# zhejz/TrafficBotsV1.5

Hardware: NVIDIA B200
Metric: closed_loop_scenario_rollout_steps_per_sec (higher is better)
Workload: dtype tf32+fp16

## Files before the change

### trafficbotsv1.5_b200/csrc/ag_frontend.cu

```cuda
#include <cuda_fp16.h>

#include "common.cuh"

namespace {

constexpr int AW = 8;
constexpr int S1 = 32 + 8, S2 = 64 + 8, SP = 128 + 8;
constexpr int OFF_W1 = 0, OFF_W2 = OFF_W1 + 64 * S1, OFF_W3 = OFF_W2 + 64 * S2, OFF_P0 = OFF_W3 + 64 * S2,
              OFF_P1 = OFF_P0 + 64 * SP, OFF_P2 = OFF_P1 + 64 * SP, W_HALVES = OFF_P2 + 64 * SP;
constexpr int N_BIAS = 6 * 64;
constexpr size_t SMEM = (size_t)W_HALVES * 2 + (N_BIAS + 8) * 4;

__device__ __forceinline__ uint32_t pack_h2(float a, float b) { return tb_pack_h2_sat(a, b); }
__device__ __forceinline__ void mma16816(float (&d)[4], const uint32_t (&a)[4], uint32_t b0, uint32_t b1) {
  asm volatile(
      "mma.sync.aligned.m16n8k16.row.col.f32.f16.f16.f32 {%0,%1,%2,%3}, {%4,%5,%6,%7}, {%8,%9}, {%0,%1,%2,%3};"
      : "+f"(d[0]), "+f"(d[1]), "+f"(d[2]), "+f"(d[3])
      : "r"(a[0]), "r"(a[1]), "r"(a[2]), "r"(a[3]), "r"(b0), "r"(b1));
}

template <int KC>
__device__ __forceinline__ void dense64(const uint32_t (&a)[KC][4], const __half* __restrict__ Ws, int stride,
                                        const float* __restrict__ bias, int g, int t, float (&c)[8][4]) {
#pragma unroll
  for (int nt = 0; nt < 8; ++nt) {
    const float2 bb = *reinterpret_cast<const float2*>(bias + nt * 8 + 2 * t);
    c[nt][0] = bb.x; c[nt][1] = bb.y; c[nt][2] = bb.x; c[nt][3] = bb.y;
    const __half* wr = Ws + (nt * 8 + g) * stride + 2 * t;
#pragma unroll
    for (int kc = 0; kc < KC; ++kc)
      mma16816(c[nt], a[kc], *reinterpret_cast<const uint32_t*>(wr + kc * 16),
               *reinterpret_cast<const uint32_t*>(wr + kc * 16 + 8));
  }
}
template <bool RELU>
__device__ __forceinline__ void c_to_a(const float (&c)[8][4], uint32_t (*a)[4], uint32_t& hm) {
#pragma unroll
  for (int kc = 0; kc < 4; ++kc) {
    auto r = [](float v) { return RELU ? fmaxf(v, 0.f) : v; };
    a[kc][0] = pack_h2(r(c[2 * kc][0]), r(c[2 * kc][1]));
    a[kc][1] = pack_h2(r(c[2 * kc][2]), r(c[2 * kc][3]));
    a[kc][2] = pack_h2(r(c[2 * kc + 1][0]), r(c[2 * kc + 1][1]));
    a[kc][3] = pack_h2(r(c[2 * kc + 1][2]), r(c[2 * kc + 1][3]));
#pragma unroll
    for (int j = 0; j < 4; ++j) tb_track_h2(hm, a[kc][j]);
  }
}
__device__ __forceinline__ void relu_colmax(float (&c)[8][4], bool v_lo, bool v_hi, float (&m)[8][2]) {
#pragma unroll
  for (int nt = 0; nt < 8; ++nt) {
#pragma unroll
    for (int r = 0; r < 4; ++r) c[nt][r] = fmaxf(c[nt][r], 0.f);
    float a = fmaxf(v_lo ? c[nt][0] : -INFINITY, v_hi ? c[nt][2] : -INFINITY);
    float b = fmaxf(v_lo ? c[nt][1] : -INFINITY, v_hi ? c[nt][3] : -INFINITY);
#pragma unroll
    for (int o = 4; o < 32; o <<= 1) {
      a = fmaxf(a, __shfl_xor_sync(TB_FULL_MASK, a, o));
      b = fmaxf(b, __shfl_xor_sync(TB_FULL_MASK, b, o));
    }
    m[nt][0] = a; m[nt][1] = b;
  }
}
__device__ __forceinline__ float pe64(int c, float x, float y, float w, const float* __restrict__ f) {
  float a;
  bool is_sin;
  if (c < 16) { a = x * f[c & 7]; is_sin = c >= 8; }
  else if (c < 32) { a = y * f[c & 7]; is_sin = c >= 24; }
  else { a = w * (float)(((c - 32) & 15) + 1); is_sin = c >= 48; }
  return is_sin ? __sinf(a) : __cosf(a);
}

__global__ void __launch_bounds__(AW * 32, 2)
ag_frontend_kernel(const uint8_t* __restrict__ hist_valid, const float* __restrict__ hist_pose,
                   const float* __restrict__ hist_motion, const float* __restrict__ ag_attr,
                   const int* __restrict__ d_step, int step_stride, int A, const float* __restrict__ freq_xy,
                   int n_ag_tot, int W, const __half* __restrict__ wblob, const float* __restrict__ bias, float* __restrict__ tok_out,
                   int ldo, float* __restrict__ tok_pose, uint8_t* __restrict__ tok_invalid,
                   const float* __restrict__ ln_g, const float* __restrict__ ln_b, __half* __restrict__ ln_out,
                   int ld_ln, unsigned int* __restrict__ sat_flag) {
  extern __shared__ __align__(16) unsigned char smem[];
  __half* sW = reinterpret_cast<__half*>(smem);
  float* sB = reinterpret_cast<float*>(smem + (size_t)W_HALVES * 2);
  for (int i = threadIdx.x; i < W_HALVES / 8; i += blockDim.x)
    reinterpret_cast<uint4*>(sW)[i] = __ldg(reinterpret_cast<const uint4*>(wblob) + i);
  for (int i = threadIdx.x; i < N_BIAS; i += blockDim.x) sB[i] = __ldg(bias + i);
  if (threadIdx.x < 8) sB[N_BIAS + threadIdx.x] = __ldg(freq_xy + threadIdx.x);
  __syncthreads();

  const int warp = threadIdx.x >> 5, lane = threadIdx.x & 31;
  const int g = lane >> 2, t = lane & 3;
  const int s_all = *d_step;
  float* fr = sB + N_BIAS;
  uint32_t hm = 0u;

  for (int ba = blockIdx.x * AW + warp; ba < n_ag_tot; ba += gridDim.x * AW) {
    const size_t hb = (size_t)ba * W;
    const int s = step_stride ? d_step[(size_t)(ba / A) * step_stride] : s_all;
    const int n_step = min(s, W);
    int last_wp = -1;
    for (int wp = W - n_step; wp < W; ++wp)
      if (hist_valid[hb + ((s - W + wp) % W)]) last_wp = wp;
    float px = 0.f, py = 0.f, pw = 0.f;
    if (last_wp >= 0) {
      const int slot = (s - W + last_wp) % W;
      px = hist_pose[(hb + slot) * 3];
      py = hist_pose[(hb + slot) * 3 + 1];
      pw = hist_pose[(hb + slot) * 3 + 2];
    }
    if (lane == 0) {
      tok_pose[(size_t)ba * 3] = px; tok_pose[(size_t)ba * 3 + 1] = py; tok_pose[(size_t)ba * 3 + 2] = pw;
      tok_invalid[ba] = last_wp < 0;
    }
    float sn, cs;
    sincosf(pw, &sn, &cs);

    bool present[2], valid[2];
    float lx[2], ly[2], lw[2], mo[2][3];
#pragma unroll
    for (int h = 0; h < 2; ++h) {
      const int wp = g + 8 * h;
      present[h] = wp < W && wp >= W - n_step;
      const int slot = present[h] ? (s - W + wp) % W : 0;
      valid[h] = present[h] && hist_valid[hb + slot];
      lx[h] = ly[h] = lw[h] = 0.f;
      mo[h][0] = mo[h][1] = mo[h][2] = 0.f;
      if (present[h]) {
        const float* hp = hist_pose + (hb + slot) * 3;
        const float dx = hp[0] - px, dy = hp[1] - py;
        lx[h] = fmaf(dx, cs, dy * sn);
        ly[h] = fmaf(dy, cs, -dx * sn);
        lw[h] = hp[2] - pw;
        const float* hm = hist_motion + (hb + slot) * 3;
        mo[h][0] = hm[0]; mo[h][1] = hm[1]; mo[h][2] = hm[2];
      }
    }
    auto attr_el = [&](int h, int col) -> float {
      if (!present[h]) return 0.f;
      if (col < 6) return __ldg(ag_attr + (size_t)ba * 6 + col);
      if (col < 9) return col == 6 ? mo[h][0] : (col == 7 ? mo[h][1] : mo[h][2]);
      if (col < 9 + W) return (col - 9) == (g + 8 * h) ? 1.f : 0.f;
      return 0.f;
    };
    uint32_t a1[2][4];
#pragma unroll
    for (int kc = 0; kc < 2; ++kc) {
      const int c0 = 16 * kc + 2 * t;
      a1[kc][0] = pack_h2(attr_el(0, c0), attr_el(0, c0 + 1));
      a1[kc][1] = pack_h2(attr_el(1, c0), attr_el(1, c0 + 1));
      a1[kc][2] = pack_h2(attr_el(0, c0 + 8), attr_el(0, c0 + 9));
      a1[kc][3] = pack_h2(attr_el(1, c0 + 8), attr_el(1, c0 + 9));
    }
    float c[8][4];
    uint32_t x[8][4];
    dense64<2>(a1, sW + OFF_W1, S1, sB, g, t, c);
    c_to_a<true>(c, x, hm);
    {
      uint32_t a2[4][4];
#pragma unroll
      for (int kc = 0; kc < 4; ++kc)
#pragma unroll
        for (int r = 0; r < 4; ++r) a2[kc][r] = x[kc][r];
      dense64<4>(a2, sW + OFF_W2, S2, sB + 64, g, t, c);
      c_to_a<true>(c, a2, hm);
      dense64<4>(a2, sW + OFF_W3, S2, sB + 128, g, t, c);
      c_to_a<false>(c, x, hm);
    }
#pragma unroll
    for (int kc = 0; kc < 4; ++kc) {
      const int c0 = 16 * kc + 2 * t;
      x[4 + kc][0] = pack_h2(pe64(c0, lx[0], ly[0], lw[0], fr), pe64(c0 + 1, lx[0], ly[0], lw[0], fr));
      x[4 + kc][1] = pack_h2(pe64(c0, lx[1], ly[1], lw[1], fr), pe64(c0 + 1, lx[1], ly[1], lw[1], fr));
      x[4 + kc][2] = pack_h2(pe64(c0 + 8, lx[0], ly[0], lw[0], fr), pe64(c0 + 9, lx[0], ly[0], lw[0], fr));
      x[4 + kc][3] = pack_h2(pe64(c0 + 8, lx[1], ly[1], lw[1], fr), pe64(c0 + 9, lx[1], ly[1], lw[1], fr));
    }
    float m[8][2];
    dense64<8>(x, sW + OFF_P0, SP, sB + 192, g, t, c);
    relu_colmax(c, valid[0], valid[1], m);
#pragma unroll
    for (int layer = 1; layer < 3; ++layer) {
      c_to_a<false>(c, x, hm);
#pragma unroll
      for (int kc = 0; kc < 4; ++kc) {
        x[4 + kc][0] = x[4 + kc][1] = pack_h2(m[2 * kc][0], m[2 * kc][1]);
        x[4 + kc][2] = x[4 + kc][3] = pack_h2(m[2 * kc + 1][0], m[2 * kc + 1][1]);
      }
      dense64<8>(x, sW + (layer == 1 ? OFF_P1 : OFF_P2), SP, sB + 192 + 64 * layer, g, t, c);
      relu_colmax(c, valid[0], valid[1], m);
    }
    float2 o = make_float2(0.f, 0.f);
#pragma unroll
    for (int nt = 0; nt < 8; ++nt)
      if (nt == g) o = make_float2(m[nt][0], m[nt][1]);
    if (last_wp < 0) o = make_float2(0.f, 0.f);
    float* op = tok_out + (size_t)ba * ldo + 8 * g + 2 * t;
    *reinterpret_cast<float2*>(op) = o;
    *reinterpret_cast<float2*>(op + 64) = o;
    if (ln_out) {
      float sum = o.x + o.y;
#pragma unroll
      for (int of = 16; of; of >>= 1) sum += __shfl_xor_sync(TB_FULL_MASK, sum, of);
      const float mean = sum * (1.f / 64.f);
      const float dx = o.x - mean, dy = o.y - mean;
      float sq = fmaf(dx, dx, dy * dy);
#pragma unroll
      for (int of = 16; of; of >>= 1) sq += __shfl_xor_sync(TB_FULL_MASK, sq, of);
      const float rstd = 1.f / sqrtf(sq * (1.f / 64.f) + 1e-5f);
      const int c0 = 8 * g + 2 * t;
      __half* lp = ln_out + (size_t)ba * ld_ln + c0;
#pragma unroll
      for (int hlf = 0; hlf < 2; ++hlf) {
        const float2 gg = *reinterpret_cast<const float2*>(ln_g + c0 + 64 * hlf);
        const float2 bb = *reinterpret_cast<const float2*>(ln_b + c0 + 64 * hlf);
        *reinterpret_cast<__half2*>(lp + 64 * hlf) = __floats2half2_rn(dx * rstd * gg.x + bb.x, dy * rstd * gg.y + bb.y);
      }
    }
  }
  tb_flag_if_sat(hm, sat_flag);
}

}

extern "C" int tb_ag_frontend_blob_halves(void) { return W_HALVES; }

extern "C" int tb_ag_frontend_ex(const uint8_t* hist_valid, const float* hist_pose, const float* hist_motion,
                                 const float* ag_attr, const int* d_step, int step_stride, const float* freq_xy, int B,
                                 int A, int W, const void* wblob, const float* bias, float* tok_out, int ldo,
                                 float* tok_pose, uint8_t* tok_invalid, const float* ln_gamma, const float* ln_beta,
                                 void* ln_out, int ld_ln, void* stream) {
  if (!hist_valid || !hist_pose || !hist_motion || !ag_attr || !d_step || !freq_xy || !wblob || !bias || !tok_out ||
      !tok_pose || !tok_invalid)
    return TB_ERR_NULL;
  if (B <= 0 || A <= 0 || W <= 0 || ldo < 128 || step_stride < 0) return TB_ERR_BAD_SHAPE;
  if (W > 16 || 9 + W > 32) return TB_ERR_UNSUPPORTED;
  if ((ldo & 1) || !tb_aligned16(wblob) || (reinterpret_cast<uintptr_t>(tok_out) & 7)) return TB_ERR_MISALIGNED;
  if (ln_out) {
    if (!ln_gamma || !ln_beta) return TB_ERR_NULL;
    if (ld_ln < 128) return TB_ERR_BAD_SHAPE;
    if ((ld_ln & 1) || (reinterpret_cast<uintptr_t>(ln_out) & 3) || (reinterpret_cast<uintptr_t>(ln_gamma) & 7) ||
        (reinterpret_cast<uintptr_t>(ln_beta) & 7))
      return TB_ERR_MISALIGNED;
  }
  static bool attr_set = false;
  if (!attr_set) {
    if (cudaFuncSetAttribute(ag_frontend_kernel, cudaFuncAttributeMaxDynamicSharedMemorySize, (int)SMEM) != cudaSuccess)
      return TB_ERR_CUDA;
    attr_set = true;
  }
  static int num_sms = 0;
  if (num_sms == 0) {
    int dev = 0;
    cudaGetDevice(&dev);
    if (cudaDeviceGetAttribute(&num_sms, cudaDevAttrMultiProcessorCount, dev) != cudaSuccess || num_sms <= 0)
      num_sms = 148;
  }
  const int n = B * A;
  const int want = (n + AW - 1) / AW;
  const int grid = want < 2 * num_sms ? want : 2 * num_sms;
  ag_frontend_kernel<<<grid, AW * 32, SMEM, static_cast<cudaStream_t>(stream)>>>(
      hist_valid, hist_pose, hist_motion, ag_attr, d_step, step_stride, A, freq_xy, n, W,
      static_cast<const __half*>(wblob), bias, tok_out, ldo, tok_pose, tok_invalid, ln_gamma, ln_beta,
      static_cast<__half*>(ln_out), ld_ln, tb_fp16_flag_ptr);
  TB_CHECK_LAUNCH();
  return TB_OK;
}

extern "C" int tb_ag_frontend(const uint8_t* hist_valid, const float* hist_pose, const float* hist_motion,
                              const float* ag_attr, const int* d_step, const float* freq_xy, int B, int A, int W,
                              const void* wblob, const float* bias, float* tok_out, int ldo, float* tok_pose,
                              uint8_t* tok_invalid, const float* ln_gamma, const float* ln_beta, void* ln_out, int ld_ln,
                              void* stream) {
  return tb_ag_frontend_ex(hist_valid, hist_pose, hist_motion, ag_attr, d_step, 0, freq_xy, B, A, W, wblob, bias, tok_out,
                           ldo, tok_pose, tok_invalid, ln_gamma, ln_beta, ln_out, ld_ln, stream);
}
```

### trafficbotsv1.5_b200/model.py

```python
import math
from typing import Dict, Optional


import torch
from torch import Tensor

from . import ops

H = 4


def fuse_attention(P: Dict[str, Tensor], prefix: str, d: int, n_head: int = H, differentiable: bool = False
                   ) -> Dict[str, Tensor]:
    if differentiable:
        f64 = lambda k: P[f"{prefix}.{k}"].double()
    else:
        f64 = lambda k: P[f"{prefix}.{k}"].detach().double().cpu()
    w_in, b_in = f64("in_proj_weight"), f64("in_proj_bias")
    w_o, b_o = f64("out_proj_weight"), f64("out_proj_bias")
    w_r, b_r = f64("linear_rpe.weight"), f64("linear_rpe.bias")
    dh = d // n_head
    d_rpe = w_r.shape[1]
    s = math.log2(math.e) / math.sqrt(dh)
    w_q, b_q = w_in[:d] * s, b_in[:d] * s
    w_rk, w_rv, b_rv = w_r[:d], w_r[d:], b_r[d:]
    w_u, b_u, w_oz = [], [], []
    for h in range(n_head):
        sl = slice(h * dh, (h + 1) * dh)
        w_u.append(w_rk[sl].T @ w_q[sl])
        b_u.append(w_rk[sl].T @ b_q[sl])
        w_oz.append(w_o[:, sl] @ w_rv[sl])
    w_qu = torch.cat([w_q] + w_u, 0)
    b_qu = torch.cat([b_q] + b_u, 0)
    out = dict(
        w_in_self=torch.cat([w_qu, w_in[d:]], 0), b_in_self=torch.cat([b_qu, b_in[d:]], 0),
        w_in_q=w_qu, b_in_q=b_qu, w_kv=w_in[d:], b_kv=b_in[d:],
        w_out=torch.cat([w_o] + w_oz, 1), b_out=b_o + w_o @ b_rv,
    )
    return {k: v.float().contiguous() for k, v in out.items()}


def head_interleave_perm(d: int = 128, n_head: int = H) -> Tensor:
    assert d == 128 and n_head == 4
    s = torch.arange(d)
    head = 2 * (s >> 6) + ((s >> 3) & 1)
    return 32 * head + 8 * ((s >> 4) & 3) + (s & 7)


def _probe_fp32(fn):
    import functools

    @functools.wraps(fn)
    def wrapped(self, *a, **k):
        if getattr(self, "_probe_heads_fp32", False) and self.precision != 0:
            saved = (self.precision, self.kv_half)
            self.precision, self.kv_half = 0, False
            try:
                return fn(self, *a, **k)
            finally:
                self.precision, self.kv_half = saved
        return fn(self, *a, **k)
    return wrapped


class HotPathModel:

    _OPT = dict(attn_il=True, ln_fused=True, chain=True)

    @property
    def opt(self) -> dict:
        if "_opt" not in self.__dict__:
            self._opt = dict(self._OPT)
        return self._opt

    def __init__(self, P: Dict[str, Tensor], cfg: dict, sizes: dict, device="cuda", precision: int = 0):
        self.cfg, self.sz, self.dev, self.precision = cfg, sizes, torch.device(device), precision
        self.d = cfg["hidden_dim"]
        self.kv_half = precision == 1 and self.d == 128
        self.W = cfg["temp_window_size"]
        self.P = {k: v.detach().to(self.dev, torch.float32).contiguous() for k, v in P.items()}
        self.fa: Dict[str, Dict[str, Tensor]] = {}
        for k in P:
            if k.endswith(".in_proj_weight"):
                p = k[: -len(".in_proj_weight")]
                self.fa[p] = {n: t.to(self.dev) for n, t in fuse_attention(P, p, self.d).items()}
        self.freq_rpe = ops.pe_freq_xy(self.d, cfg["pose_rpe"]["theta_xy"], self.dev)
        self.freq_ag = ops.pe_freq_xy(self.d // 2, cfg["ag_encoder"]["pose_emb"]["theta_xy"], self.dev)
        self.act_w0 = torch.cat([self.P[f"action_head.mlp_mean.{t}.fc_layers.0.weight"] for t in range(3)], 0)
        self.act_b0 = torch.cat([self.P[f"action_head.mlp_mean.{t}.fc_layers.0.bias"] for t in range(3)], 0)
        self.act_w4 = torch.block_diag(*[self.P[f"action_head.mlp_mean.{t}.fc_layers.4.weight"] for t in range(3)]
                                       ).contiguous()
        self.act_b4 = torch.cat([self.P[f"action_head.mlp_mean.{t}.fc_layers.4.bias"] for t in range(3)], 0)

    @classmethod
    def from_state_dict(cls, sd: Dict[str, Tensor], d_model: int, theta_xy: float = 1e3, device="cuda",
                        precision: int = 0) -> "HotPathModel":
        self = cls.__new__(cls)
        self.cfg, self.sz, self.dev, self.precision = None, None, torch.device(device), precision
        self.d, self.W = d_model, None
        self.kv_half = precision == 1 and d_model == 128
        self.P = {k: v.detach().to(self.dev, torch.float32).contiguous() for k, v in sd.items()}
        self.fa = {}
        for k in sd:
            if k.endswith("in_proj_weight"):
                p = k[: -len(".in_proj_weight")] if k.endswith(".in_proj_weight") else ""
                P = sd if p else {f".{n}": t for n, t in sd.items()}
                self.fa[p] = {n: t.to(self.dev) for n, t in fuse_attention(P, p, d_model).items()}
        self.freq_rpe = ops.pe_freq_xy(d_model, theta_xy, self.dev)
        return self

    @property
    def gp(self) -> int:
        return 3 if (self.precision == 0 and getattr(self, "fp32_tc", True)) else self.precision

    def lin(self, x, wname, relu=False, **kw):
        return ops.linear(x, self.P[f"{wname}.weight"], self.P[f"{wname}.bias"], relu=relu, precision=self.gp,
                          **kw)

    def ln(self, x, name, half: bool = False):
        return ops.layernorm(x, self.P[f"{name}.weight"], self.P[f"{name}.bias"],
                             out_dtype=torch.float16 if half else torch.float32)

    @property
    def kv_il(self) -> bool:
        return self.kv_half and self.opt["attn_il"]

    def _proj(self, x: Tensor, key: str, w: Tensor, b: Tensor, il_blocks=(), **kw):
        if x.dtype == torch.float16:
            if il_blocks and self.kv_il:
                w, b = self._interleaved(key, w, b, il_blocks)
                key += ".il"
            return ops.linear(x, self._half(key, w), b, precision=2, **kw)
        return ops.linear(x, w, b, precision=self.gp, **kw)

    def _interleaved(self, key: str, w: Tensor, b: Tensor, blocks):
        if not hasattr(self, "_w_il"):
            self._w_il = {}
        if key not in self._w_il:
            rows = torch.arange(w.shape[0], device=w.device)
            perm = head_interleave_perm(self.d).to(w.device)
            for r0 in blocks:
                rows[r0:r0 + self.d] = r0 + perm
            self._w_il[key] = (w[rows].contiguous(), b[rows].contiguous())
        return self._w_il[key]

    def mlp(self, x, prefix, idxs, end_act, **last_kw):
        for n, i in enumerate(idxs):
            last = n == len(idxs) - 1
            x = self.lin(x, f"{prefix}.fc_layers.{i}", relu=(not last) or end_act, **(last_kw if last else {}))
        return x

    def pointnet(self, x: Tensor, row_invalid: Tensor, G: int, Lg: int, prefix: str) -> Tensor:
        half = self.d // 2
        h = self.lin(x, f"{prefix}.mlp_layers.0.fc_layers.0", relu=True)
        for i in (1, 2):
            m = ops.pointnet_pool(h, row_invalid, G, Lg, 1)
            w_l, w_r = self._pointnet_split(prefix, i)
            gb = ops.linear(m, w_r, self.P[f"{prefix}.mlp_layers.{i}.fc_layers.0.bias"], precision=self.gp)
            h = ops.linear(h, w_l, gb, relu=True, bias_group=Lg, precision=self.gp)
        return ops.pointnet_pool(h, row_invalid, G, Lg, 2)

    def _pointnet_split(self, prefix: str, i: int):
        key = f"{prefix}.{i}"
        if not hasattr(self, "_pn_split"):
            self._pn_split = {}
        if key not in self._pn_split:
            w = self.P[f"{prefix}.mlp_layers.{i}.fc_layers.0.weight"]
            half = w.shape[1] // 2
            self._pn_split[key] = (w[:, :half].contiguous(), w[:, half:].contiguous())
        return self._pn_split[key]

    def kv_table(self, feat: Tensor, layer_prefix: str, norm: str, attn: str = "attn", out: Optional[Tensor] = None
                 ) -> Tensor:
        f = self.fa[f"{layer_prefix}.{attn}"]
        x = self.ln(feat, f"{layer_prefix}.{norm}", half=self.kv_half)
        if self.kv_half:
            tbl = out if out is not None else torch.empty(x.shape[0], 2 * self.d, dtype=torch.float16, device=x.device)
            self._proj(x, f"{layer_prefix}.{attn}.w_kv", f["w_kv"], f["b_kv"], out_h=tbl, col_h=0,
                       il_blocks=(0, self.d))
            return tbl
        return ops.linear(x, f["w_kv"], f["b_kv"], precision=self.gp, out=out)

    def _in_self(self, f, x, K, key=""):
        nq = self.d + H * self.d
        if self.kv_half:
            row = torch.empty(x.shape[0], nq + 2 * self.d, dtype=torch.float16, device=x.device)
            self._proj(x, f"{key}.w_in_self", f["w_in_self"], f["b_in_self"], out_h=row, col_h=0,
                       il_blocks=(0, nq, nq + self.d))
            return row[:, :nq], row[:, nq:]
        proj = ops.linear(x, f["w_in_self"], f["b_in_self"], precision=self.gp)
        return proj, proj[:, nq:]

    def _in_q(self, f, x, key=""):
        if self.kv_half:
            qu = torch.empty(x.shape[0], self.d + H * self.d, dtype=torch.float16, device=x.device)
            self._proj(x, f"{key}.w_in_q", f["w_in_q"], f["b_in_q"], out_h=qu, col_h=0, il_blocks=(0,))
            return qu
        return ops.linear(x, f["w_in_q"], f["b_in_q"], precision=self.gp)

    def _attend(self, fa, proj, B, S, kv0, T0, div0, K0, knn, kv1=None, T1=0, div1=1, K1=0):
        d = self.d
        if torch.is_grad_enabled() and any(t is not None and t.requires_grad for t in (proj, kv0, kv1)):
            from . import autograd as AG
            return AG.knarpe_attn(proj[:, :d + H * d], kv0, T0, div0, K0, knn["idx"], knn["inv"], knn["rel"],
                                  self.freq_rpe, B, S, d, H, kv1=kv1, T1=T1, div1=div1, K1=K1,
                                  fast_trig=self.precision == 1)
        return ops.knarpe_attn(proj[:, :d], proj[:, d:d + H * d], kv0, T0, div0, K0, knn["idx"], knn["inv"],
                               knn.get("rel"), self.freq_rpe, B, S, d, H, kv1=kv1, T1=T1, div1=div1, K1=K1,
                               emb=knn.get("emb"), fast_trig=self.precision == 1, interleaved=self.kv_il,
                               out_dtype=torch.float16 if self.kv_half else torch.float32)

    def _half(self, key: str, w: Tensor) -> Tensor:
        if not hasattr(self, "_w_half"):
            self._w_half = {}
        if key not in self._w_half:
            self._w_half[key] = w.to(torch.float16).contiguous()
        return self._w_half[key]

    @property
    def chain_fused(self) -> bool:
        return self.opt["chain"]

    def _ffn_program(self, p: str, ldy: int, ln_next: Optional[str]):
        if not hasattr(self, "_chain"):
            self._chain = {}
        key = ("ffn", p, ldy, ln_next)
        if key not in self._chain:
            d = self.d
            w1 = self._half(f"{p}.linear1", self.P[f"{p}.linear1.weight"])
            w2 = self._half(f"{p}.linear2", self.P[f"{p}.linear2.weight"])
            nh = w1.shape[0] // d
            assert w1.shape == (nh * d, d) and w2.shape == (d, nh * d) and nh <= 4
            q = ops.ChainProgram(self.dev, n_buf=nh)
            q.load(0, d, 0, f16=True)
            hb = [(t + 1) % nh for t in range(nh)]
            for t in range(nh):
                q.gemm(w1, [0], self.P[f"{p}.linear1.bias"], n0=t * d, relu=True, out_buf=hb[t])
            ln = dict(ln_out=4, ld_ln=d, ln_gamma=self.P[f"{ln_next}.weight"], ln_beta=self.P[f"{ln_next}.bias"]) if ln_next else {}
            q.gemm(w2, hb, self.P[f"{p}.linear2.bias"], res=1, ldr=d, mask_post=2, out_g=3, ldg=ldy, **ln)
            self._chain[key] = q.finish()
        return self._chain[key]

    def _heads_program(self):
        if not hasattr(self, "_chain"):
            self._chain = {}
        if "heads" not in self._chain:
            d = self.d
            hw = lambda n: self._half(n, self.P[f"{n}.weight"])
            b = lambda n: self.P[f"{n}.bias"]
            q = ops.ChainProgram(self.dev, n_buf=4)
            q.load(1, d, 1)
            q.load(0, 2 * d, 0)
            n = "navi_encoder.mlp_pe.fc_layers.0"
            q.gemm(hw(n), [1], b(n), res=2, ldr=d, out_buf=2)
            for i, (src_b, dst_b) in zip((0, 3, 6), ((2, 1), (1, 2), (2, 1))):
                n = f"add_navi.mlp_in.fc_layers.{i}"
                q.gemm(hw(n), [src_b], b(n), relu=True, out_buf=dst_b, mask_post=3 if i == 6 else -1)
            n = "add_navi.mlp.fc_layers.0"
            q.gemm(hw(n), [0, 1], b(n), relu=True, out_buf=2)
            n = "add_navi.mlp.fc_layers.3"
            q.gemm(hw(n), [2], b(n), relu=True, out_buf=3)
            n = "add_navi.mlp.fc_layers.6"
            q.gemm(hw(n), [3], b(n), relu=True, mask_pre=3, res=0, ldr=2 * d, out_buf=0, out_g=4, ldg=2 * d)
            q.load(4, 2 * d, 1, src_col=d)
            n = "add_latent.mlp.fc_layers.0"
            q.gemm(hw(n), [0, 1], b(n), relu=True, out_buf=2)
            n = "add_latent.mlp.fc_layers.3"
            q.gemm(hw(n), [2], b(n), relu=True, out_buf=3)
            n = "add_latent.mlp.fc_layers.6"
            q.gemm(hw(n), [3], b(n), relu=True, mask_pre=5, res=4, ldr=2 * d, out_buf=0)
            w0 = self._half("action_head.w0", self.act_w0)
            for t in range(3):
                q.gemm(w0, [0], self.act_b0, n0=t * d, relu=True, out_buf=1 + t)
            for t in range(3):
                n = f"action_head.mlp_mean.{t}.fc_layers.2"
                q.gemm(hw(n), [1 + t], b(n), relu=True, out_buf=1 + t)
            q.gemm(self._half("action_head.w4", self.act_w4), [1, 2, 3], self.act_b4, out_g=6, ldg=6, n_valid=6)
            self._chain["heads"] = q.finish()
        return self._chain["heads"]

    @property
    def ln_fused(self) -> bool:
        return self.kv_half and self.d == 128 and self.opt["ln_fused"]

    def _out_proj(self, p: str, f: dict, o: Tensor, nv: Tensor, res: Tensor, ln_next: Optional[str] = None):
        if o.dtype == torch.float16:
            w = self._half(f"{p}.w_out", f["w_out"])
            if ln_next is not None and self.ln_fused:
                return ops.linear_ln(o, w, f["b_out"], self.P[f"{ln_next}.weight"], self.P[f"{ln_next}.bias"], mask_pre=nv,
                                     res=res, precision=2)
            y = ops.linear(o, w, f["b_out"], mask_pre=nv, res=res, precision=2)
        else:
            y = ops.linear(o, f["w_out"], f["b_out"], mask_pre=nv, res=res, precision=self.gp)
        return y if ln_next is None else (y, self.ln(y, ln_next, half=self.kv_half))

    def tf_layer(self, p: str, mode: str, src: Tensor, src_inv: Tensor, B: int, S: int, knn_self: dict,
                 cross: Optional[dict] = None, out: Optional[Tensor] = None, before_self=None, before_cross=None,
                 ln_in: Optional[Tensor] = None, ln_next: Optional[str] = None):
        d, pr = self.d, self.precision
        if mode == "dec_cross_attn":
            f = self.fa[f"{p}.attn_src"]
            x0 = ln_in if ln_in is not None else self.ln(src, f"{p}.norm_src", half=self.kv_half)
            proj, kv = self._in_self(f, x0, knn_self["idx"].shape[-1], f"{p}.attn_src")
            if before_self is not None:
                before_self()
            o, nv = self._attend(f, proj, B, S, kv, S, 1, knn_self["idx"].shape[-1], knn_self)
            src, x1 = self._out_proj(f"{p}.attn_src", f, o, nv, src, ln_next=f"{p}.norm1")
            f = self.fa[f"{p}.attn"]
            proj = self._in_q(f, x1, f"{p}.attn")
            if before_cross is not None:
                before_cross()
            o, nv = self._attend(f, proj, B, S, cross["kv0"], cross["T0"], cross["div0"], cross["K0"], cross,
                                 cross.get("kv1"), cross.get("T1", 0), cross.get("div1", 1), cross.get("K1", 0))
            src, x2 = self._out_proj(f"{p}.attn", f, o, nv, src, ln_next=f"{p}.norm2")
        else:
            f = self.fa[f"{p}.attn"]
            x0 = ln_in if ln_in is not None else self.ln(src, f"{p}.norm1", half=self.kv_half)
            proj, kv = self._in_self(f, x0, knn_self["idx"].shape[-1], f"{p}.attn")
            o, nv = self._attend(f, proj, B, S, kv, S, 1, knn_self["idx"].shape[-1], knn_self)
            src, x2 = self._out_proj(f"{p}.attn", f, o, nv, src, ln_next=f"{p}.norm2")
        if self.kv_half:
            h = torch.empty(x2.shape[0], self.P[f"{p}.linear1.weight"].shape[0], dtype=torch.float16, device=x2.device)
            self._proj(x2, f"{p}.linear1", self.P[f"{p}.linear1.weight"], self.P[f"{p}.linear1.bias"], relu=True, out_h=h,
                       col_h=0)
            w2 = self._half(f"{p}.linear2", self.P[f"{p}.linear2.weight"])
            if ln_next is not None and self.ln_fused:
                return ops.linear_ln(h, w2, self.P[f"{p}.linear2.bias"], self.P[f"{ln_next}.weight"],
                                     self.P[f"{ln_next}.bias"], res=src, mask_post=src_inv, out=out, precision=2)
            y = ops.linear(h, w2, self.P[f"{p}.linear2.bias"], res=src, mask_post=src_inv, out=out, precision=2)
        else:
            h = self.lin(x2, f"{p}.linear1", relu=True)
            y = self.lin(h, f"{p}.linear2", res=src, mask_post=src_inv, out=out)
        return y if ln_next is None else (y, self.ln(y, ln_next, half=self.kv_half))

    def tf_stack(self, prefix: str, n_layer: int, mode: str, tok: Tensor, layer_kw, ln_in: Optional[Tensor] = None
                 ) -> Tensor:
        first = "norm_src" if mode == "dec_cross_attn" else "norm1"
        for i in range(n_layer):
            args, kw = layer_kw(i)
            nxt = f"{prefix}.{i + 1}.{first}" if (i + 1 < n_layer and self.ln_fused) else None
            r = self.tf_layer(f"{prefix}.{i}", mode, tok, *args, ln_in=ln_in, ln_next=nxt, **kw)
            tok, ln_in = r if nxt is not None else (r, None)
        return tok

    def map_encoder(self, mp_valid: Tensor, mp_attr: Tensor, mp_pose: Tensor) -> Dict[str, Tensor]:
        d, sz = self.d, self.sz
        n_sc, n_mp, Ln = mp_valid.shape
        tok_pose = mp_pose[:, :, 0].contiguous()
        tok_inv = ~mp_valid[:, :, 0]
        c, s = torch.cos(tok_pose[..., 2]), torch.sin(tok_pose[..., 2])
        rot = torch.stack([torch.stack([c, -s], -1), torch.stack([s, c], -1)], -2)
        xy = torch.matmul(mp_pose[..., :2] - tok_pose[:, :, None, :2], rot)
        yaw = mp_pose[..., 2] - tok_pose[..., 2:3]
        pe7 = _encode_polyline(xy, torch.stack([yaw.cos(), yaw.sin()], -1))
        attr = torch.cat([mp_attr[:, :, None, :].expand(-1, -1, Ln, -1),
                          torch.eye(Ln, device=self.dev)[None, None].expand(n_sc, n_mp, -1, -1)], -1)
        M = n_sc * n_mp * Ln
        x = torch.empty(M, d, device=self.dev)
        x[:, d - 7:] = pe7.reshape(M, 7)
        self.mlp(attr.reshape(M, -1).contiguous(), "mp_encoder.input_encoder.mlp", (0, 2, 4), False, out=x[:, : d - 7])
        tok = self.pointnet(x, (~mp_valid).reshape(-1).contiguous(), n_sc * n_mp, Ln, "mp_encoder.pl_encoder")
        idx, inv, rel = ops.knn_select(tok_pose, tok_inv, tok_pose, tok_inv, sz["k_mp2mp"], sz["dl_mp"])
        knn = dict(idx=idx, inv=inv, rel=rel)
        flat_inv = tok_inv.reshape(-1).contiguous()
        tok = self.tf_stack("mp_encoder.tf_mp2mp.layers", self.cfg["mp_encoder"]["n_layer_tf"], "enc_self_attn", tok,
                            lambda i: ((flat_inv, n_sc, n_mp, knn), {}))
        return dict(mp_token_invalid=tok_inv.contiguous(), mp_token_feature=tok.view(n_sc, n_mp, d),
                    mp_token_pose=tok_pose, knn_mp2mp=knn, **self.sorted_map(tok_pose, tok_inv))

    @staticmethod
    def sorted_map(tok_pose: Tensor, tok_inv: Tensor) -> Dict[str, Tensor]:
        order = torch.argsort(tok_pose[..., 0], dim=1)
        return dict(mp_sorted_pose=torch.gather(tok_pose, 1, order[..., None].expand(-1, -1, 3)).contiguous(),
                    mp_sorted_invalid=torch.gather(tok_inv, 1, order).contiguous(),
                    mp_sorted_index=order.to(torch.int32).contiguous())

    def tl_pre_compute(self, tl_valid: Tensor, tl_attr: Tensor, tl_pose: Tensor, mp: Dict[str, Tensor]) -> dict:
        sz, d = self.sz, self.d
        n_sc, n_tl = tl_valid.shape
        n_mp = mp["mp_token_pose"].shape[1]
        inv = (~tl_valid).contiguous()
        tl_pose = tl_pose.contiguous()
        feat2d = mp["mp_token_feature"].reshape(n_sc * n_mp, d)
        attr = ops.gather_rows(mp["mp_token_feature"].contiguous(), tl_attr.to(torch.int32).reshape(-1).contiguous(),
                               n_tl)
        i1, m1, r1 = ops.knn_select(tl_pose, inv, tl_pose, inv, sz["k_tl2tl"], sz["dl_tl"])
        i2, m2, r2 = ops.knn_select(tl_pose, inv, mp["mp_token_pose"], mp["mp_token_invalid"], sz["k_tl2mp"],
                                    sz["dl_tl"])
        kv = [self.kv_table(feat2d, f"tl_encoder.tf_tl2tlmp.layers.{i}", "norm_tgt")
              for i in range(self.cfg["tl_encoder"]["n_layer_tf"])]
        W = self.W
        return dict(tl_token_invalid=inv, tl_token_pose=tl_pose, tl_token_attr=attr,
                    tl_attr_rows=attr.view(n_sc * n_tl, 1, d).expand(-1, W, -1).reshape(-1, d).contiguous(),
                    knn_self=dict(idx=i1, inv=m1, rel=r1),
                    cross=[dict(kv0=kv[i], T0=n_mp, div0=1, K0=sz["k_tl2mp"], idx=i2, inv=m2, rel=r2)
                           for i in range(len(kv))], n_sc=n_sc, n_tl=n_tl)

    def tl_forward(self, hist_tl: Tensor, d_step: Tensor, tl: dict, out_feat: Optional[Tensor] = None,
                   out_logits: Optional[Tensor] = None, with_logits: bool = True):
        from . import lib as L
        Bt, n_tl, W, d = tl["n_sc"], tl["n_tl"], self.W, self.d
        M = Bt * n_tl * W
        attr = torch.empty(M, 5 + W, device=self.dev)
        row_inv = torch.empty(M, dtype=torch.bool, device=self.dev)
        L.check(L.load().tb_tl_featurize_ex(L.ptr(hist_tl), L.ptr(ops._u8(tl["tl_token_invalid"])), L.ptr(d_step),
                                            1 if d_step.numel() > 1 else 0, Bt, n_tl, W, L.ptr(attr), 5 + W,
                                            L.ptr(ops._u8(row_inv)), L.stream()), "tb_tl_featurize_ex")
        ops._count()
        x = self.mlp(attr, "tl_encoder.input_encoder.mlp", (0, 2, 4), False, res=tl["tl_attr_rows"])
        tok = self.pointnet(x, row_inv, Bt * n_tl, W, "tl_encoder.temp_encoder")
        flat_inv = tl["tl_token_invalid"].reshape(-1)
        nl = self.cfg["tl_encoder"]["n_layer_tf"]
        tok = self.tf_stack("tl_encoder.tf_tl2tlmp.layers", nl, "dec_cross_attn", tok,
                            lambda i: ((flat_inv, Bt, n_tl, tl["knn_self"], tl["cross"][i]),
                                       dict(out=out_feat if i == nl - 1 else None)))
        if not with_logits:
            return tok, None
        tok_in = tok.detach() if getattr(self, "detach_tl_feature", False) else tok
        logits = self.mlp(tok_in, "tl_state_predictor.mlp", (0, 2, 4), False, out=out_logits)
        return tok, logits

    def ag_static(self, mp: Dict[str, Tensor]) -> list:
        n_sc, n_mp, d = mp["mp_token_feature"].shape
        feat2d = mp["mp_token_feature"].reshape(n_sc * n_mp, d)
        return [self.kv_table(feat2d, f"ag_encoder.tf_ag2agmptl.layers.{i}", "norm_tgt")
                for i in range(self.cfg["ag_encoder"]["n_layer_tf"])]

    def ag_forward(self, st: dict, mp: Dict[str, Tensor], kv_mp: list, tl: dict, tl_feat: Tensor, R: int,
                   out: Optional[Tensor] = None, aux: Optional[dict] = None, before_tl=None, knn_stream=None,
                   knn_stream2=None, kv_tl: Optional[list] = None, tl_pose_div: Optional[int] = None) -> Tensor:
        from . import lib as L
        sz, d, W = self.sz, self.d, self.W
        B, A = st["B"], st["A"]
        n_mp, n_tl = mp["mp_token_pose"].shape[1], tl["n_tl"]
        tl_div = B // (tl_feat.shape[0] // n_tl)
        M, MW = B * A, B * A * W
        tok_pose = torch.empty(B, A, 3, device=self.dev)
        tok_inv = torch.empty(B, A, dtype=torch.bool, device=self.dev)
        fused = self.kv_half and W <= 16 and d == 128
        hist = (L.ptr(st["hist_valid"]), L.ptr(st["hist_pose"]), L.ptr(st["hist_motion"]), L.ptr(st["ag_attr"]),
                L.ptr(st["d_step"]), L.ptr(self.freq_ag), B, A, W)
        per_row_step = st["d_step"].numel() > 1
        stride = 1 if per_row_step else 0
        if fused:
            L.check(L.load().tb_ag_featurize_ex(*hist[:5], stride, *hist[5:], L.ptr(tok_pose), L.ptr(ops._u8(tok_inv)),
                                                None, None, 0, None, 0, L.stream()), "tb_ag_featurize_ex")
        else:
            row_inv = torch.empty(MW, dtype=torch.bool, device=self.dev)
            attr = torch.empty(MW, 9 + W, device=self.dev)
            x = torch.empty(MW, d, device=self.dev)
            L.check(L.load().tb_ag_featurize_ex(*hist[:5], stride, *hist[5:], L.ptr(tok_pose),
                                                L.ptr(ops._u8(tok_inv)), L.ptr(ops._u8(row_inv)), L.ptr(attr), 9 + W,
                                                L.ptr(x[:, d // 2:]), d, L.stream()), "tb_ag_featurize_ex")
        ops._count()
        Kc, Ka = sz["k_ag2mp"] + sz["k_ag2tl"], sz["k_ag2ag"]
        i_aa = torch.empty(B, A, Ka, dtype=torch.int32, device=self.dev)
        m_aa = torch.empty(B, A, Ka, dtype=torch.bool, device=self.dev)
        r_aa = torch.empty(B, A, Ka, 3, device=self.dev)
        cidx = torch.empty(B, A, Kc, dtype=torch.int32, device=self.dev)
        cinv = torch.empty(B, A, Kc, dtype=torch.bool, device=self.dev)
        crel = torch.empty(B, A, Kc, 3, device=self.dev)

        def select_self():
            ops.knn_select(tok_pose, tok_inv, tok_pose, tok_inv, Ka, sz["dl_ag"], out=(i_aa, m_aa, r_aa))

        def select_cross():
            if "knn_state" in st and "mp_sorted_pose" in mp:
                ops.knn_select(tok_pose, tok_inv, mp["mp_sorted_pose"], mp["mp_sorted_invalid"], sz["k_ag2mp"],
                               sz["dl_ag"], tgt_div=R, out=(cidx, cinv, crel), koff=0,
                               index_map=mp["mp_sorted_index"], row_state=st["knn_state"], sorted_by_x=True)
            else:
                ops.knn_select(tok_pose, tok_inv, mp["mp_token_pose"], mp["mp_token_invalid"], sz["k_ag2mp"],
                               sz["dl_ag"], tgt_div=R, out=(cidx, cinv, crel), koff=0)
            ops.knn_select(tok_pose, tok_inv, tl["tl_token_pose"], tl["tl_token_invalid"], sz["k_ag2tl"], sz["dl_ag"],
                           tgt_div=tl_pose_div or tl_div, out=(cidx, cinv, crel), koff=sz["k_ag2mp"],
                           row_state=st.get("knn_state_tl"))

        main = torch.cuda.current_stream()
        join_self = join_cross = None
        if knn_stream is not None:
            s2 = knn_stream2 if knn_stream2 is not None else knn_stream
            s2.wait_stream(main)
            with torch.cuda.stream(s2):
                select_self()
            knn_stream.wait_stream(main)
            with torch.cuda.stream(knn_stream):
                select_cross()
            join_self = lambda: main.wait_stream(s2)
            join_cross = lambda: main.wait_stream(knn_stream)
        if fused:
            blob, bias = self._ag_frontend_weights()
            tok = torch.empty(M, d, device=self.dev)
            tp2, ti2 = torch.empty_like(tok_pose), torch.empty_like(tok_inv)
            ln0 = None
            if self.ln_fused:
                ln0 = torch.empty(M, d, dtype=torch.float16, device=self.dev)
                nm = "ag_encoder.tf_ag2agmptl.layers.0.norm_src"
                ln_args = (L.ptr(self.P[f"{nm}.weight"]), L.ptr(self.P[f"{nm}.bias"]), L.ptr(ln0), d)
            else:
                ln_args = (None, None, None, 0)
            L.check(L.load().tb_ag_frontend_ex(*hist[:5], stride, *hist[5:], L.ptr(blob), L.ptr(bias), L.ptr(tok), d,
                                               L.ptr(tp2), L.ptr(ops._u8(ti2)), *ln_args, L.stream()),
                    "tb_ag_frontend_ex")
            ops._count()
        else:
            ln0 = None
            self.mlp(attr, "ag_encoder.input_encoder.mlp", (0, 2, 4), False, out=x[:, : d // 2])
            tok = self.pointnet(x, row_inv, M, W, "ag_encoder.temp_encoder")
        if knn_stream is None:
            select_self()
            select_cross()
        knn_self = dict(idx=i_aa, inv=m_aa, rel=r_aa)
        flat_inv = tok_inv.reshape(-1)
        nl = self.cfg["ag_encoder"]["n_layer_tf"]
        if aux is not None:
            aux.update(tok_pose=tok_pose, tok_inv=tok_inv, tok0=tok, knn_self=knn_self, cidx=cidx, cinv=cinv, crel=crel)
        if before_tl is not None and kv_tl is None:
            before_tl()

        def join_first_cross():
            if join_cross is not None:
                join_cross()
            if before_tl is not None and kv_tl is not None:
                before_tl()

        def layer_kw(i):
            p = f"ag_encoder.tf_ag2agmptl.layers.{i}"
            kv1 = kv_tl[i] if kv_tl is not None else self.kv_table(tl_feat, p, "norm_tgt")
            cross = dict(kv0=kv_mp[i], T0=n_mp, div0=R, K0=sz["k_ag2mp"], kv1=kv1, T1=n_tl, div1=tl_div,
                         K1=sz["k_ag2tl"], idx=cidx, inv=cinv, rel=crel)
            return (flat_inv, B, A, knn_self, cross), dict(out=out if i == nl - 1 else None,
                                                           before_self=join_self if i == 0 else None,
                                                           before_cross=join_first_cross if i == 0 else None)

        tok = self.tf_stack("ag_encoder.tf_ag2agmptl.layers", nl, "dec_cross_attn", tok, layer_kw, ln_in=ln0)
        return tok

    def ag_tl_tables(self, tl_feat: Tensor, out: Optional[list] = None) -> list:
        return [self.kv_table(tl_feat, f"ag_encoder.tf_ag2agmptl.layers.{i}", "norm_tgt",
                              out=out[i] if out is not None else None)
                for i in range(self.cfg["ag_encoder"]["n_layer_tf"])]

    def navi_predictor(self, ag_valid: Tensor, ag_attr: Tensor, ag_motion: Tensor, ag_pose: Tensor,
                       mp: Dict[str, Tensor], ag_type: Tensor, mp_type: Tensor, scene_chunk: int = 4) -> Tensor:
        d, W = self.d, self.W
        n_sc, A, n_step = ag_valid.shape
        if n_step > W:
            ag_valid, ag_motion, ag_pose, n_step = ag_valid[:, :, -W:], ag_motion[:, :, -W:], ag_pose[:, :, -W:], W
        tok_valid = ag_valid.any(-1)
        last = n_step - 1 - torch.max(ag_valid.flip(2).to(torch.uint8), dim=2)[1]
        tok_pose = torch.gather(ag_pose, 2, last[:, :, None, None].expand(-1, -1, 1, 3)).squeeze(2)
        tok_pose = tok_pose.masked_fill(~tok_valid[..., None], 0.0).contiguous()
        M, MW = n_sc * A, n_sc * A * n_step
        attr = torch.cat([ag_attr[:, :, None, :].expand(-1, -1, n_step, -1), ag_motion,
                          torch.eye(W, device=self.dev)[None, None, -n_step:].expand(n_sc, A, -1, -1)], -1)
        x = torch.empty(MW, d, device=self.dev)
        self.mlp(attr.reshape(MW, -1).contiguous(), "navi_predictor.input_encoder.mlp", (0, 2, 4), False,
                 out=x[:, : d // 2])
        ops.pose_emb(ag_pose.reshape(MW, 3), self.freq_ag, d // 2, frame=tok_pose, frame_div=n_step, out=x[:, d // 2:])
        tok = self.pointnet(x, (~ag_valid).reshape(-1).contiguous(), M, n_step, "navi_predictor.temp_encoder")
        pr = "navi_predictor.mlp.fc_layers"
        w0 = self.P[f"{pr}.0.weight"]
        a_part = ops.linear(tok, w0[:, :d].contiguous(), self.P[f"{pr}.0.bias"], precision=self.gp)
        w_mr = w0[:, d:].contiguous()
        n_mp = mp["mp_token_pose"].shape[1]
        logits = torch.empty(n_sc, A, n_mp, device=self.dev)
        for s0 in range(0, n_sc, scene_chunk):
            ns = min(scene_chunk, n_sc - s0)
            Pn = ns * A * n_mp
            X = torch.empty(Pn, 2 * d, device=self.dev)
            X[:, :d].view(ns, A, n_mp, d).copy_(mp["mp_token_feature"][s0:s0 + ns, None])
            pose_rows = mp["mp_token_pose"][s0:s0 + ns, None].expand(-1, A, -1, -1).reshape(Pn, 3)
            ops.pose_emb(pose_rows, self.freq_rpe, d, frame=tok_pose[s0:s0 + ns], frame_div=n_mp, out=X[:, d:])
            h = ops.linear(X, w_mr, a_part[s0 * A:(s0 + ns) * A], bias_group=n_mp, precision=self.gp)
            h = ops.layernorm(h, self.P[f"{pr}.1.weight"], self.P[f"{pr}.1.bias"], relu=True, out=h)
            h = self.lin(h, f"{pr}.3")
            h = ops.layernorm(h, self.P[f"{pr}.4.weight"], self.P[f"{pr}.4.bias"], relu=True, out=h)
            logits[s0:s0 + ns] = self.lin(h, f"{pr}.6").view(ns, A, n_mp)
        mp_mask = mp["mp_token_invalid"] | ~(mp_type[:, :, :5].any(-1))
        inv = (mp_mask.unsqueeze(1) | (ag_type[:, :, [0]] & mp_type[:, :, 3].unsqueeze(1))
               | (ag_type[:, :, [1]] & mp_type[:, :, :4].any(-1).unsqueeze(1))
               | (ag_type[:, :, [2]] & mp_type[:, :, :3].any(-1).unsqueeze(1)))
        logits = logits.masked_fill(inv, float("-inf"))
        return logits.masked_fill((~tok_valid).unsqueeze(-1) | inv.all(-1, keepdim=True), 0.0)

    def _ag_frontend_weights(self):
        if not hasattr(self, "_ag_front"):
            from . import lib as L
            n = L.load().tb_ag_frontend_blob_halves()
            blob = torch.zeros(n, dtype=torch.float16, device=self.dev)
            names = [f"ag_encoder.input_encoder.mlp.fc_layers.{i}" for i in (0, 2, 4)] + \
                    [f"ag_encoder.temp_encoder.mlp_layers.{i}.fc_layers.0" for i in range(3)]
            off = 0
            for nm, stride in zip(names, (40, 72, 72, 136, 136, 136)):
                w = self.P[f"{nm}.weight"]
                assert w.shape[0] == 64 and w.shape[1] <= stride - 8, w.shape
                blob[off:off + 64 * stride].view(64, stride)[:, : w.shape[1]] = w.to(torch.float16)
                off += 64 * stride
            assert off == n
            bias = torch.cat([self.P[f"{nm}.bias"] for nm in names]).contiguous()
            self._ag_front = (blob, bias)
        return self._ag_front

    @_probe_fp32
    def navi_static(self, mp: Dict[str, Tensor], dest_idx: Tensor, R: int) -> dict:
        B, A = dest_idx.shape
        flat = dest_idx.reshape(-1).contiguous()
        f = ops.gather_rows(mp["mp_token_feature"].contiguous(), flat, A, R)
        pose = ops.gather_rows(mp["mp_token_pose"].contiguous(), flat, A, R)
        return dict(feat=self.lin(f, "navi_encoder.mlp_mp.fc_layers.0"), pose=pose)

    @_probe_fp32
    def latent_static(self, navi: dict, st: dict) -> None:
        d = self.d
        M = st["latent"].shape[0]
        cat = torch.zeros(M, 2 * d, device=self.dev)
        self.mlp(st["latent"], "add_latent.mlp_in", (0, 3, 6), True, mask_post=st["latent_invalid"].reshape(-1),
                 out=cat[:, d:])
        navi["latent_cat"] = cat
        navi["latent_feat"] = True

    @_probe_fp32
    def heads(self, x_cat: Tensor, st: dict, navi: dict) -> Tensor:
        d = self.d
        M = x_cat.shape[0]
        pe = ops.pose_emb(navi["pose"], self.freq_rpe, d, frame=st["pose"], frame_div=1)
        if self.kv_half and self.chain_fused and d == 128 and "latent_cat" in navi and x_cat.is_contiguous():
            act = torch.empty(M, 6, device=self.dev)
            self._heads_program().run([x_cat, pe, navi["feat"], ops._u8(st["navi_invalid"]).reshape(-1), navi["latent_cat"],
                                       ops._u8(st["latent_invalid"]).reshape(-1), act], M)
            return act
        nf = self.lin(pe, "navi_encoder.mlp_pe.fc_layers.0", res=navi["feat"])
        x_cat2 = navi["latent_cat"] if "latent_cat" in navi else torch.empty(M, 2 * d, device=self.dev)
        for prefix, z, zinv, cat_in, cat_out in (("add_navi", nf, st["navi_invalid"], x_cat, x_cat2[:, :d]),
                                                 ("add_latent", st["latent"], st["latent_invalid"], x_cat2, None)):
            zinv = zinv.reshape(-1)
            if prefix == "add_latent" and "latent_feat" in navi:
                cat_in = navi["latent_cat"]
            else:
                self.mlp(z, f"{prefix}.mlp_in", (0, 3, 6), True, mask_post=zinv, out=cat_in[:, d:])
            h = self.mlp(cat_in, f"{prefix}.mlp", (0, 3, 6), True, mask_pre=zinv, res=cat_in[:, :d], out=cat_out)
        if self.kv_half:
            h0 = torch.empty(M, 3 * d, dtype=torch.float16, device=self.dev)
            ops.linear(h, self.act_w0, self.act_b0, relu=True, precision=1, out_h=h0, col_h=0)
            h1 = torch.empty_like(h0)
            for t in range(3):
                nm = f"action_head.mlp_mean.{t}.fc_layers.2"
                ops.linear(h0[:, t * d:(t + 1) * d], self._half(nm, self.P[f"{nm}.weight"]), self.P[f"{nm}.bias"],
                           relu=True, precision=2, out_h=h1[:, t * d:(t + 1) * d], col_h=0)
            return ops.linear(h1, self._half("action_head.w4", self.act_w4), self.act_b4, precision=2)
        h0 = ops.linear(h, self.act_w0, self.act_b0, relu=True, precision=self.gp)
        h1 = torch.empty_like(h0)
        for t in range(3):
            self.lin(h0[:, t * d:(t + 1) * d], f"action_head.mlp_mean.{t}.fc_layers.2", relu=True,
                     out=h1[:, t * d:(t + 1) * d])
        return ops.linear(h1, self.act_w4, self.act_b4, precision=self.gp)


def _encode_polyline(pos: Tensor, dirv: Tensor) -> Tensor:
    eps = torch.finfo(pos.dtype).eps
    proj = (-pos * dirv).sum(-1) / ((dirv * dirv).sum(-1) + eps)
    closest = pos + proj.clamp(0, 1).unsqueeze(-1) * dirv
    r = torch.norm(closest, dim=-1, keepdim=True)
    dn = torch.norm(dirv, dim=-1, keepdim=True)
    return torch.cat([r, closest / (r + eps), dirv / (dn + eps), dn,
                      torch.norm(pos + dirv - closest, dim=-1, keepdim=True)], -1)
```

Before: 134,400.

## Use atomic work-stealing in agent frontend and launch cross kNN after it

```diff
diff --git a/profiles/inproj_time.py b/profiles/inproj_time.py
--- /dev/null
+++ b/profiles/inproj_time.py
@@ -0,0 +1,23 @@
+import sys, os, json
+sys.path.insert(0, os.path.dirname(os.path.dirname(os.path.abspath(__file__))))
+import torch
+import tbpkg
+from trafficbotsv1_5_b200 import ops
+M = 61440
+torch.manual_seed(0)
+x = torch.randn(M, 128, device="cuda").half()
+res = {}
+for N in (256, 640, 896):
+    w = (torch.randn(N, 128, device="cuda") * 0.05).half()
+    b = torch.randn(N, device="cuda")
+    out = torch.empty(M, N, dtype=torch.float16, device="cuda")
+    for _ in range(20):
+        ops.linear(x, w, b, precision=2, out_h=out, col_h=0)
+    torch.cuda.synchronize()
+    e0, e1 = torch.cuda.Event(True), torch.cuda.Event(True)
+    e0.record()
+    for _ in range(200):
+        ops.linear(x, w, b, precision=2, out_h=out, col_h=0)
+    e1.record(); torch.cuda.synchronize()
+    res[N] = e0.elapsed_time(e1) / 200 * 1e3
+print(json.dumps({f"proj_N{n}_us": round(v, 2) for n, v in res.items()}))
diff --git a/trafficbotsv1.5_b200/csrc/ag_frontend.cu b/trafficbotsv1.5_b200/csrc/ag_frontend.cu
--- a/trafficbotsv1.5_b200/csrc/ag_frontend.cu
+++ b/trafficbotsv1.5_b200/csrc/ag_frontend.cu
@@ -69,6 +69,8 @@
   else { a = w * (float)(((c - 32) & 15) + 1); is_sin = c >= 48; }
   return is_sin ? __sinf(a) : __cosf(a);
 }
+
+__device__ unsigned int g_ag_work[2];
 
 __global__ void __launch_bounds__(AW * 32, 2)
 ag_frontend_kernel(const uint8_t* __restrict__ hist_valid, const float* __restrict__ hist_pose,
@@ -93,7 +95,11 @@
   float* fr = sB + N_BIAS;
   uint32_t hm = 0u;
 
-  for (int ba = blockIdx.x * AW + warp; ba < n_ag_tot; ba += gridDim.x * AW) {
+  for (;;) {
+    unsigned int next = 0u;
+    if (lane == 0) next = atomicAdd(&g_ag_work[0], 1u);
+    const int ba = (int)__shfl_sync(TB_FULL_MASK, next, 0);
+    if (ba >= n_ag_tot) break;
     const size_t hb = (size_t)ba * W;
     const int s = step_stride ? d_step[(size_t)(ba / A) * step_stride] : s_all;
     const int n_step = min(s, W);
@@ -216,6 +222,15 @@
     }
   }
   tb_flag_if_sat(hm, sat_flag);
+  __syncthreads();
+  if (threadIdx.x == 0) {
+    __threadfence();
+    if (atomicAdd(&g_ag_work[1], 1u) == gridDim.x - 1) {
+      g_ag_work[0] = 0u;
+      g_ag_work[1] = 0u;
+      __threadfence();
+    }
+  }
 }
 
 }
diff --git a/trafficbotsv1.5_b200/model.py b/trafficbotsv1.5_b200/model.py
--- a/trafficbotsv1.5_b200/model.py
+++ b/trafficbotsv1.5_b200/model.py
@@ -483,11 +483,7 @@
             s2.wait_stream(main)
             with torch.cuda.stream(s2):
                 select_self()
-            knn_stream.wait_stream(main)
-            with torch.cuda.stream(knn_stream):
-                select_cross()
             join_self = lambda: main.wait_stream(s2)
-            join_cross = lambda: main.wait_stream(knn_stream)
         if fused:
             blob, bias = self._ag_frontend_weights()
             tok = torch.empty(M, d, device=self.dev)
@@ -507,7 +503,12 @@
             ln0 = None
             self.mlp(attr, "ag_encoder.input_encoder.mlp", (0, 2, 4), False, out=x[:, : d // 2])
             tok = self.pointnet(x, row_inv, M, W, "ag_encoder.temp_encoder")
-        if knn_stream is None:
+        if knn_stream is not None:
+            knn_stream.wait_stream(main)
+            with torch.cuda.stream(knn_stream):
+                select_cross()
+            join_cross = lambda: main.wait_stream(knn_stream)
+        else:
             select_self()
             select_cross()
         knn_self = dict(idx=i_aa, inv=m_aa, rel=r_aa)
```

Result: no change. 133,600, median of 6 (-0.6%).
